# apache/arrow-rs

Measured on NVIDIA H100. Metric: Mrows/sec filter+take+add on 1e9-row Int64/Float64; % HBM roofline, higher is better.
Workload: dtype i64 (filter/take/sum) + f64 (add)

## Files before the change

### arrow-rs_b200/csrc/common.cuh

```cuda
#pragma once

#include <cuda_runtime.h>
#include <stdint.h>
#include <string.h>

#include <functional>
#include <unordered_map>
#include <vector>

#include "../../include/arrow_cuda.h"

#define ACU_FULL_MASK 0xffffffffu

enum {
  RES_COUNT = 0,
  RES_ERR_INDEX = 1,
  RES_AUX0 = 2,
  RES_AUX1 = 3,
  RES_AUX2 = 4,
  RES_AUX3 = 5,
  RES_ERR2 = 6,
  RES_SLOTS = 16,
  RES_BLOCKS = 64
};

struct acu_ctx {
  int device = 0;
  int sm_count = 0;
  cudaStream_t stream = nullptr;
  cudaEvent_t ev_start = nullptr, ev_stop = nullptr;
  acu_error_detail err{};
  int64_t launches = 0;
  int64_t bytes_allocated = 0;
  std::unordered_map<void *, size_t> allocs;
  std::unordered_map<const void *, int> occupancy;
  unsigned long long *d_res = nullptr;
  unsigned long long *h_res = nullptr;
  bool res_clean = false;
  int res_dirty_blocks = RES_BLOCKS;
  bool async_on = false;
  int async_blocks = 0;
  std::vector<std::function<acu_status(const unsigned long long *)>> async_fin;
  std::vector<int> async_blk;
  void *d_scratch = nullptr;
  size_t scratch_bytes = 0;
  void *nccl_comm = nullptr;
  int rank = 0, world = 1;
  cudaEvent_t tev[ACU_TIMER_SLOTS][2] = {};
  static constexpr int KEV_PAIRS = 64;
  cudaEvent_t kev[KEV_PAIRS][2] = {};
  int kev_class[KEV_PAIRS] = {};
  int kev_pending = 0;
  double kstat_ms[ACU_K_CLASSES] = {};
  int64_t kstat_n[ACU_K_CLASSES] = {};
};

void acu_kstats_drain(acu_ctx *ctx);
int acu_kstats_begin(acu_ctx *ctx, int cls);
void acu_kstats_end(acu_ctx *ctx, int slot);

acu_status acu_fail(acu_ctx *ctx, acu_status st, int64_t index, uint64_t lhs, uint64_t rhs,
                    uint64_t len, const char *fmt, ...) __attribute__((format(printf, 7, 8)));
acu_status acu_cuda_fail(acu_ctx *ctx, cudaError_t e, const char *what);
acu_status acu_scratch(acu_ctx *ctx, size_t bytes, void **out);
acu_status acu_res_reset(acu_ctx *ctx);
acu_status acu_res_fetch(acu_ctx *ctx);
acu_status acu_res_reset_n(acu_ctx *ctx, int blocks);
acu_status acu_res_fetch_n(acu_ctx *ctx, int blocks);
int acu_call_begin(acu_ctx *ctx, acu_status *st);
acu_status acu_call_end(acu_ctx *ctx, int block, std::function<acu_status(const unsigned long long *)> fin);
static inline unsigned long long *acu_dres(acu_ctx *ctx, int block) { return ctx->d_res + (size_t)block * RES_SLOTS; }
static inline const unsigned long long *acu_hres(const acu_ctx *ctx, int block) { return ctx->h_res + (size_t)block * RES_SLOTS; }
int64_t acu_resolve_null_count(acu_ctx *ctx, const acu_array *a, acu_status *st);

#define ACU_CUDA(ctx, expr)                                         \
  do {                                                              \
    cudaError_t _e = (expr);                                        \
    if (_e != cudaSuccess) return acu_cuda_fail((ctx), _e, #expr);  \
  } while (0)

#define ACU_ENTER(ctx)                                                                      \
  do {                                                                                      \
    cudaError_t _e = cudaSetDevice((ctx)->device);                                          \
    if (_e != cudaSuccess) return acu_cuda_fail((ctx), _e, "cudaSetDevice");                \
  } while (0)

#define ACU_TRY(expr)                  \
  do {                                 \
    acu_status _s = (expr);            \
    if (_s != ACU_OK) return _s;       \
  } while (0)

#define ACU_LAUNCH(ctx, kernel, grid, block, smem, ...)                            \
  do {                                                                             \
    kernel<<<(grid), (block), (smem), (ctx)->stream>>>(__VA_ARGS__);               \
    (ctx)->launches++;                                                             \
    cudaError_t _e = cudaGetLastError();                                           \
    if (_e != cudaSuccess) return acu_cuda_fail((ctx), _e, "launch " #kernel);     \
  } while (0)

#define ACU_LAUNCH_TIMED(ctx, cls, kernel, grid, block, smem, ...)                 \
  do {                                                                             \
    int _slot = acu_kstats_begin((ctx), (cls));                                    \
    kernel<<<(grid), (block), (smem), (ctx)->stream>>>(__VA_ARGS__);               \
    (ctx)->launches++;                                                             \
    cudaError_t _e = cudaGetLastError();                                           \
    acu_kstats_end((ctx), _slot);                                                  \
    if (_e != cudaSuccess) return acu_cuda_fail((ctx), _e, "launch " #kernel);     \
  } while (0)

static inline int acu_dtype_size(acu_dtype t) {
  switch (t) {
    case ACU_I8: case ACU_U8: return 1;
    case ACU_I16: case ACU_U16: return 2;
    case ACU_I32: case ACU_U32: case ACU_F32: return 4;
    default: return 8;
  }
}
static inline bool acu_dtype_is_float(acu_dtype t) { return t == ACU_F32 || t == ACU_F64; }
static inline bool acu_dtype_is_signed(acu_dtype t) { return t <= ACU_I64; }
static inline const char *acu_dtype_name(acu_dtype t) {
  static const char *n[] = {"Int8", "Int16", "Int32", "Int64", "UInt8", "UInt16", "UInt32", "UInt64", "Float32", "Float64"};
  return n[(int)t];
}

static inline int acu_grid(const acu_ctx *ctx, int64_t work_items, int per_sm) {
  int64_t g = (int64_t)ctx->sm_count * per_sm;
  if (g > work_items) g = work_items;
  if (g < 1) g = 1;
  return (int)g;
}

#ifdef __CUDACC__
template <class K>
static inline int acu_wave_grid(acu_ctx *ctx, K kernel, int block, size_t smem, int64_t work_blocks) {
  const void *key = reinterpret_cast<const void *>(kernel);
  auto it = ctx->occupancy.find(key);
  int per_sm;
  if (it == ctx->occupancy.end()) {
    per_sm = 0;
    if (cudaOccupancyMaxActiveBlocksPerMultiprocessor(&per_sm, kernel, block, smem) != cudaSuccess || per_sm < 1) per_sm = 1;
    ctx->occupancy[key] = per_sm;
  } else {
    per_sm = it->second;
  }
  return acu_grid(ctx, work_blocks, per_sm * 8);
}


__device__ __forceinline__ uint64_t ld_bits64(const uint8_t *__restrict__ base, int64_t pos, int64_t end) {
  int64_t n = end - pos;
  if (n <= 0) return 0ull;
  uintptr_t addr = (uintptr_t)base + (uintptr_t)(pos >> 3);
  uintptr_t al = addr & ~(uintptr_t)7;
  unsigned shift = (unsigned)((addr & 7) << 3) + (unsigned)(pos & 7);
  const uint64_t *p = reinterpret_cast<const uint64_t *>(al);
  uint64_t w = __ldg(p) >> shift;
  if (shift != 0 && (int64_t)(64 - shift) < n) w |= __ldg(p + 1) << (64 - shift);
  if (n < 64) w &= (~0ull) >> (64 - n);
  return w;
}

__device__ __forceinline__ uint32_t ld_bits32(const uint8_t *__restrict__ base, int64_t pos, int64_t end) {
  int64_t n = end - pos;
  if (n <= 0) return 0u;
  uintptr_t addr = (uintptr_t)base + (uintptr_t)(pos >> 3);
  uintptr_t al = addr & ~(uintptr_t)3;
  unsigned shift = (unsigned)((addr & 3) << 3) + (unsigned)(pos & 7);
  const uint32_t *p = reinterpret_cast<const uint32_t *>(al);
  uint32_t w = __ldg(p) >> shift;
  if (shift != 0 && (int64_t)(32 - shift) < n) w |= __ldg(p + 1) << (32 - shift);
  if (n < 32) w &= (~0u) >> (32 - n);
  return w;
}

__device__ __forceinline__ uint32_t ld_bit(const uint8_t *__restrict__ base, int64_t pos) {
  return (__ldg(base + (pos >> 3)) >> (pos & 7)) & 1u;
}

__device__ __forceinline__ uint4 ld_stream16(const void *p) {
  uint4 r;
  asm volatile("ld.global.nc.L1::no_allocate.v4.u32 {%0,%1,%2,%3}, [%4];"
               : "=r"(r.x), "=r"(r.y), "=r"(r.z), "=r"(r.w) : "l"(p));
  return r;
}
__device__ __forceinline__ void st_stream16(void *p, uint4 v) {
  asm volatile("st.global.cs.v4.u32 [%0], {%1,%2,%3,%4};" ::"l"(p), "r"(v.x), "r"(v.y), "r"(v.z), "r"(v.w) : "memory");
}
__device__ __forceinline__ uint64_t ld_stream8(const void *p) {
  uint64_t r;
  asm volatile("ld.global.nc.L1::no_allocate.u64 %0, [%1];" : "=l"(r) : "l"(p));
  return r;
}
__device__ __forceinline__ void st_stream8(void *p, uint64_t v) {
  asm volatile("st.global.cs.u64 [%0], %1;" ::"l"(p), "l"(v) : "memory");
}

template <class T> __device__ __forceinline__ T warp_sum(T v) {
#pragma unroll
  for (int o = 16; o > 0; o >>= 1) v += __shfl_xor_sync(ACU_FULL_MASK, v, o);
  return v;
}

__device__ __forceinline__ uint64_t splitmix64(uint64_t x) {
  x += 0x9E3779B97F4A7C15ull;
  x = (x ^ (x >> 30)) * 0xBF58476D1CE4E5B9ull;
  x = (x ^ (x >> 27)) * 0x94D049BB133111EBull;
  return x ^ (x >> 31);
}

__device__ __forceinline__ int64_t total_key(double x) {
  int64_t b = __double_as_longlong(x);
  return b ^ (int64_t)((uint64_t)(b >> 63) >> 1);
}
__device__ __forceinline__ int32_t total_key(float x) {
  int32_t b = __float_as_int(x);
  return b ^ (int32_t)((uint32_t)(b >> 31) >> 1);
}
#endif
```

### arrow-rs_b200/csrc/elementwise.cu

```cuda
#include <stdio.h>

#include <limits>
#include <type_traits>

#include "bitmap.cuh"

namespace {

template <class T, int EPL> struct alignas(EPL * sizeof(T) == 16 ? 16 : sizeof(T)) Pack { T v[EPL]; };

template <class T, int EPL>
__device__ __forceinline__ Pack<T, EPL> pack_load(const T *p) {
  Pack<T, EPL> r;
  if constexpr (EPL * sizeof(T) == 16) {
    uint4 x = ld_stream16(p);
    r = *reinterpret_cast<Pack<T, EPL> *>(&x);
  } else {
    static_assert(EPL == 1, "scalar path");
    r.v[0] = __ldg(p);
  }
  return r;
}
template <class T, int EPL>
__device__ __forceinline__ void pack_store(T *p, Pack<T, EPL> r) {
  if constexpr (EPL * sizeof(T) == 16) {
    st_stream16(p, *reinterpret_cast<uint4 *>(&r));
  } else {
    *p = r.v[0];
  }
}

__device__ __forceinline__ uint64_t ones_to(int64_t row, int64_t n) {
  int64_t k = n - row;
  return k >= 64 ? ~0ull : (k <= 0 ? 0ull : ((~0ull) >> (64 - k)));
}

enum { CLS_WRAP = 0, CLS_CHECKED = 1, CLS_DIVREM = 2 };
enum { OP_ADD = 0, OP_SUB = 1, OP_MUL = 2, OP_DIV = 3, OP_REM = 4, OP_NEG = 5 };

template <class T> struct is_fp { static constexpr bool value = std::is_floating_point<T>::value; };

__device__ __forceinline__ double fp_add(double a, double b) { return __dadd_rn(a, b); }
__device__ __forceinline__ double fp_sub(double a, double b) { return __dsub_rn(a, b); }
__device__ __forceinline__ double fp_mul(double a, double b) { return __dmul_rn(a, b); }
__device__ __forceinline__ double fp_div(double a, double b) { return __ddiv_rn(a, b); }
__device__ __forceinline__ double fp_rem(double a, double b) { return fmod(a, b); }
__device__ __forceinline__ float fp_add(float a, float b) { return __fadd_rn(a, b); }
__device__ __forceinline__ float fp_sub(float a, float b) { return __fsub_rn(a, b); }
__device__ __forceinline__ float fp_mul(float a, float b) { return __fmul_rn(a, b); }
__device__ __forceinline__ float fp_div(float a, float b) { return __fdiv_rn(a, b); }
__device__ __forceinline__ float fp_rem(float a, float b) { return fmodf(a, b); }

template <class T, int CLS>
__device__ __forceinline__ bool apply_op(int op, T l, T r, T &o) {
  if constexpr (is_fp<T>::value) {
    if constexpr (CLS == CLS_DIVREM) {
      o = (op == OP_DIV) ? fp_div(l, r) : fp_rem(l, r);
    } else {
      o = (op == OP_ADD) ? fp_add(l, r) : (op == OP_SUB) ? fp_sub(l, r) : (op == OP_MUL) ? fp_mul(l, r) : -r;
    }
    return false;
  } else {
    using U = typename std::make_unsigned<T>::type;
    constexpr bool SIGNED = std::is_signed<T>::value;
    if constexpr (CLS == CLS_WRAP) {
      U a = (U)l, b = (U)r;
      o = (T)((op == OP_ADD) ? (U)(a + b) : (op == OP_SUB) ? (U)(a - b) : (op == OP_MUL) ? (U)(a * b) : (U)((U)0 - b));
      return false;
    } else if constexpr (CLS == CLS_CHECKED) {
      if constexpr (sizeof(T) < 8) {
        using W = typename std::conditional<SIGNED, int64_t, uint64_t>::type;
        W a = (W)l, b = (W)r;
        W w = (op == OP_ADD) ? a + b : (op == OP_SUB) ? a - b : (op == OP_MUL) ? a * b : (W)0 - b;
        o = (T)w;
        if constexpr (SIGNED) return w < (W)std::numeric_limits<T>::min() || w > (W)std::numeric_limits<T>::max();
        else return (op == OP_SUB) ? (a < b) : (op == OP_NEG ? false : w > (W)std::numeric_limits<T>::max());
      } else if constexpr (SIGNED) {
        int64_t a = l, b = r;
        if (op == OP_NEG) { a = 0; }
        if (op == OP_ADD) {
          int64_t s = (int64_t)((uint64_t)a + (uint64_t)b);
          o = s;
          return ((a ^ s) & (b ^ s)) < 0;
        } else if (op == OP_MUL) {
          int64_t lo = (int64_t)((uint64_t)a * (uint64_t)b);
          int64_t hi = __mul64hi(a, b);
          o = lo;
          return hi != (lo >> 63);
        } else {
          int64_t s = (int64_t)((uint64_t)a - (uint64_t)b);
          o = s;
          return ((a ^ b) & (a ^ s)) < 0;
        }
      } else {
        uint64_t a = l, b = r;
        if (op == OP_ADD) { o = a + b; return o < a; }
        if (op == OP_MUL) { o = a * b; return __umul64hi(a, b) != 0; }
        if (op == OP_NEG) { o = (uint64_t)0 - b; return false; }
        o = a - b;
        return a < b;
      }
    } else {
      o = 0;
      if (r == 0) return true;
      if constexpr (SIGNED) {
        if (r == (T)-1) {
          if (op == OP_DIV) {
            if (l == std::numeric_limits<T>::min()) return true;
            o = (T)(-l);
          }
          return false;
        }
      }
      o = (op == OP_DIV) ? (T)(l / r) : (T)(l % r);
      return false;
    }
  }
}

template <class T>
struct ArithParams {
  const T *a, *b;
  T *out;
  int64_t n;
  const uint8_t *av, *bv;
  int64_t aoff, boff;
  uint64_t *out_valid;
  unsigned long long *res;
  int op;
  int a_scalar, b_scalar;
  int zero_nulls;
};

template <class T, int CLS, int EPL>
__global__ void __launch_bounds__(256, (CLS == CLS_WRAP ? 4 : 3)) k_arith(const ArithParams<T> p) {
  constexpr int R = (32 * EPL > 64) ? 32 * EPL : 64;
  constexpr int LPS = R / (32 * EPL);
  constexpr int U = (LPS >= 2) ? 2 : 4;
  constexpr int GROUP = U * R;
  constexpr int SG = 2048;
  constexpr int GPS = SG / GROUP;
  constexpr bool fallible = (CLS != CLS_WRAP) && !is_fp<T>::value;
  const int lane = threadIdx.x & 31;
  const int64_t warp = ((int64_t)blockIdx.x * blockDim.x + threadIdx.x) >> 5;
  const int64_t nwarps = ((int64_t)gridDim.x * blockDim.x) >> 5;
  const int64_t n = p.n;
  const int64_t sgroups = n / SG;
  const bool has_valid = p.out_valid != nullptr;
  T sa = T(), sb = T();
  if (p.a_scalar) sa = __ldg(p.a);
  if (p.b_scalar) sb = __ldg(p.b);
  unsigned valid_cnt = 0;
  unsigned long long err = ~0ull;

  for (int64_t sg = warp; sg < sgroups; sg += nwarps) {
    const int64_t sbase = sg * SG;
    uint64_t vw = ~0ull;
    if (has_valid) {
      const int64_t row = sbase + lane * 64;
      if (p.av) vw &= ld_bits64(p.av, p.aoff + row, p.aoff + n);
      if (p.bv) vw &= ld_bits64(p.bv, p.boff + row, p.boff + n);
      p.out_valid[row >> 6] = vw;
      valid_cnt += __popcll(vw);
    }
#pragma unroll 1
    for (int gi = 0; gi < GPS; ++gi) {
      const int64_t base = sbase + gi * GROUP;
      const T *__restrict__ pa = p.a + base + lane * EPL;
      const T *__restrict__ pb = p.b + base + lane * EPL;
      Pack<T, EPL> va[U * LPS], vb[U * LPS];
#pragma unroll
      for (int k = 0; k < U * LPS; ++k) {
        if (!p.a_scalar) va[k] = pack_load<T, EPL>(pa + k * 32 * EPL);
        if (!p.b_scalar) vb[k] = pack_load<T, EPL>(pb + k * 32 * EPL);
      }
      T *__restrict__ po = p.out + base + lane * EPL;
#pragma unroll
      for (int k = 0; k < U * LPS; ++k) {
        uint32_t bits = ~0u;
        if (fallible && p.zero_nulls) {
          const int pos = gi * GROUP + k * 32 * EPL + lane * EPL;
          const uint64_t w = __shfl_sync(ACU_FULL_MASK, vw, pos >> 6);
          bits = (uint32_t)(w >> (pos & 63));
        }
        Pack<T, EPL> o;
#pragma unroll
        for (int e = 0; e < EPL; ++e) {
          const T l = p.a_scalar ? sa : va[k].v[e];
          const T r = p.b_scalar ? sb : vb[k].v[e];
          T x;
          const bool bad = apply_op<T, CLS>(p.op, l, r, x);
          if (fallible) {
            if (!((bits >> e) & 1u)) x = T();
            else if (bad) {
              const unsigned long long i = (unsigned long long)(base + k * 32 * EPL + lane * EPL + e);
              err = i < err ? i : err;
            }
          }
          o.v[e] = x;
        }
        pack_store<T, EPL>(po + k * 32 * EPL, o);
      }
    }
  }

  if (warp == 0) {
    for (int64_t row = sgroups * SG; row < n; row += 64) {
      uint64_t vw = ones_to(row, n);
      if (has_valid) {
        if (p.av) vw &= ld_bits64(p.av, p.aoff + row, p.aoff + n);
        if (p.bv) vw &= ld_bits64(p.bv, p.boff + row, p.boff + n);
        if (lane == 0) { p.out_valid[row >> 6] = vw; valid_cnt += __popcll(vw); }
      }
#pragma unroll
      for (int h = 0; h < 2; ++h) {
        const int64_t i = row + h * 32 + lane;
        if (i >= n) continue;
        const T l = p.a_scalar ? sa : __ldg(p.a + i);
        const T r = p.b_scalar ? sb : __ldg(p.b + i);
        T x;
        const bool bad = apply_op<T, CLS>(p.op, l, r, x);
        if (fallible) {
          const bool live = !p.zero_nulls || ((vw >> (h * 32 + lane)) & 1ull);
          if (!live) x = T();
          else if (bad) err = (unsigned long long)i < err ? (unsigned long long)i : err;
        }
        p.out[i] = x;
      }
    }
  }
  if (has_valid) {
    valid_cnt = warp_sum(valid_cnt);
    if (lane == 0 && valid_cnt) atomicAdd(p.res + RES_COUNT, (unsigned long long)valid_cnt);
  }
  if (fallible && err != ~0ull) atomicMin(p.res + RES_ERR_INDEX, err);
}

template <class T, int CLS>
acu_status launch_arith(acu_ctx *ctx, const ArithParams<T> &p) {
  constexpr int EPLV = 16 / sizeof(T);
  bool aligned = ((uintptr_t)p.out % 16 == 0) && (p.a_scalar || (uintptr_t)p.a % 16 == 0) &&
                 (p.b_scalar || (uintptr_t)p.b % 16 == 0);
  if (aligned) {
    int64_t blocks = (p.n / 2048 + 1 + 7) / 8;
    ACU_LAUNCH_TIMED(ctx, ACU_K_ARITH, (k_arith<T, CLS, EPLV>), acu_wave_grid(ctx, k_arith<T, CLS, EPLV>, 256, 0, blocks), 256, 0, p);
  } else {
    int64_t blocks = (p.n / 2048 + 1 + 7) / 8;
    ACU_LAUNCH_TIMED(ctx, ACU_K_ARITH, (k_arith<T, CLS, 1>), acu_wave_grid(ctx, k_arith<T, CLS, 1>, 256, 0, blocks), 256, 0, p);
  }
  return ACU_OK;
}

const char *op_symbol(acu_arith_op op) {
  switch (op) {
    case ACU_ADD_WRAPPING: case ACU_ADD: return "+";
    case ACU_SUB_WRAPPING: case ACU_SUB: return "-";
    case ACU_MUL_WRAPPING: case ACU_MUL: return "*";
    case ACU_DIV: return "/";
    default: return "%";
  }
}

template <class T> void fmt_native(char *buf, size_t n, T v) {
  if constexpr (std::is_floating_point<T>::value) snprintf(buf, n, "%.17g", (double)v);
  else if constexpr (std::is_signed<T>::value) snprintf(buf, n, "%lld", (long long)v);
  else snprintf(buf, n, "%llu", (unsigned long long)v);
}
template <class T> uint64_t bits_of(T v) { uint64_t b = 0; memcpy(&b, &v, sizeof(T)); return b; }

template <class T>
acu_status arith_error(acu_ctx *ctx, acu_arith_op op, bool is_neg, const acu_array *a, const acu_array *b, int64_t idx) {
  T l = T(), r = T();
  if (a) ACU_CUDA(ctx, cudaMemcpyAsync(&l, static_cast<const T *>(a->values) + (a->is_scalar ? 0 : idx), sizeof(T), cudaMemcpyDeviceToHost, ctx->stream));
  ACU_CUDA(ctx, cudaMemcpyAsync(&r, static_cast<const T *>(b->values) + (b->is_scalar ? 0 : idx), sizeof(T), cudaMemcpyDeviceToHost, ctx->stream));
  ACU_CUDA(ctx, cudaStreamSynchronize(ctx->stream));
  char ls[40], rs[40];
  fmt_native(ls, sizeof ls, l);
  fmt_native(rs, sizeof rs, r);
  if (is_neg)
    return acu_fail(ctx, ACU_ERR_ARITHMETIC_OVERFLOW, idx, bits_of(r), 0, 0, "Overflow happened on: - %s", rs);
  if ((op == ACU_DIV || op == ACU_REM) && r == T())
    return acu_fail(ctx, ACU_ERR_DIVIDE_BY_ZERO, idx, bits_of(l), bits_of(r), 0, "Divide by zero error");
  return acu_fail(ctx, ACU_ERR_ARITHMETIC_OVERFLOW, idx, bits_of(l), bits_of(r), 0,
                  "Overflow happened on: %s %s %s", ls, op_symbol(op), rs);
}

acu_status set_new_null(acu_ctx *ctx, int64_t len, size_t value_bytes, acu_array_out *out) {
  if (value_bytes) ACU_CUDA(ctx, cudaMemsetAsync(out->values, 0, value_bytes, ctx->stream));
  if (len) ACU_CUDA(ctx, cudaMemsetAsync(out->validity, 0, acu_bitmap_bytes(len), ctx->stream));
  ACU_CUDA(ctx, cudaStreamSynchronize(ctx->stream));
  out->len = len;
  out->has_validity = 1;
  out->null_count = len;
  return ACU_OK;
}

template <class T>
acu_status arith_typed(acu_ctx *ctx, acu_arith_op op, const acu_array *a, const acu_array *b, acu_array_out *out) {
  const bool checked = !is_fp<T>::value && (op == ACU_ADD || op == ACU_SUB || op == ACU_MUL || op == ACU_DIV || op == ACU_REM);
  const bool a_s = a->is_scalar != 0, b_s = b->is_scalar != 0;
  acu_status st;
  ArithParams<T> p{};
  p.a = static_cast<const T *>(a->values);
  p.b = static_cast<const T *>(b->values);
  p.out = static_cast<T *>(out->values);
  p.res = ctx->d_res;
  p.a_scalar = a_s && !b_s;
  p.b_scalar = b_s && !a_s;
  switch (op) {
    case ACU_ADD_WRAPPING: case ACU_ADD: p.op = OP_ADD; break;
    case ACU_SUB_WRAPPING: case ACU_SUB: p.op = OP_SUB; break;
    case ACU_MUL_WRAPPING: case ACU_MUL: p.op = OP_MUL; break;
    case ACU_DIV: p.op = OP_DIV; break;
    default: p.op = OP_REM; break;
  }
  out->has_validity = 0;
  out->null_count = 0;
  int64_t len;
  if (a_s != b_s) {
    const acu_array *s = a_s ? a : b, *arr = a_s ? b : a;
    len = arr->len;
    int64_t snc = acu_resolve_null_count(ctx, s, &st);
    ACU_TRY(st);
    if (snc != 0) return set_new_null(ctx, len, (size_t)len * sizeof(T), out);
    out->len = len;
    if (len == 0) { out->has_validity = arr->validity != nullptr; return ACU_OK; }
    if (arr->validity) {
      (a_s ? p.bv : p.av) = arr->validity;
      (a_s ? p.boff : p.aoff) = arr->validity_offset;
      p.out_valid = reinterpret_cast<uint64_t *>(out->validity);
      p.zero_nulls = checked;
    }
  } else {
    if (a->len != b->len)
      return acu_fail(ctx, ACU_ERR_COMPUTE, -1, 0, 0, 0,
                      checked ? "Cannot perform a binary operation on arrays of different length"
                              : "Cannot perform binary operation on arrays of different length");
    len = a->len;
    out->len = len;
    if (len == 0) return ACU_OK;
    int64_t an = acu_resolve_null_count(ctx, a, &st);
    ACU_TRY(st);
    int64_t bn = acu_resolve_null_count(ctx, b, &st);
    ACU_TRY(st);
    if (a->validity && b->validity && (an > 0 || bn > 0)) {
      p.av = a->validity; p.aoff = a->validity_offset;
      p.bv = b->validity; p.boff = b->validity_offset;
    } else if (a->validity && !b->validity && an > 0) {
      p.av = a->validity; p.aoff = a->validity_offset;
    } else if (b->validity && !a->validity && bn > 0) {
      p.bv = b->validity; p.boff = b->validity_offset;
    }
    if (p.av || p.bv) {
      p.out_valid = reinterpret_cast<uint64_t *>(out->validity);
      p.zero_nulls = checked;
    }
  }
  p.n = len;
  const int blk = acu_call_begin(ctx, &st);
  ACU_TRY(st);
  p.res = acu_dres(ctx, blk);
  if (is_fp<T>::value) {
    if (op == ACU_DIV || op == ACU_REM) ACU_TRY((launch_arith<T, CLS_DIVREM>(ctx, p)));
    else ACU_TRY((launch_arith<T, CLS_WRAP>(ctx, p)));
  } else if (op == ACU_DIV || op == ACU_REM) {
    ACU_TRY((launch_arith<T, CLS_DIVREM>(ctx, p)));
  } else if (checked) {
    ACU_TRY((launch_arith<T, CLS_CHECKED>(ctx, p)));
  } else {
    ACU_TRY((launch_arith<T, CLS_WRAP>(ctx, p)));
  }
  const acu_array ca = *a, cb = *b;
  const bool has_valid = p.out_valid != nullptr;
  return acu_call_end(ctx, blk, [ctx, op, checked, ca, cb, has_valid, len, out](const unsigned long long *h) -> acu_status {
    if (checked && h[RES_ERR_INDEX] != ~0ull) return arith_error<T>(ctx, op, false, &ca, &cb, (int64_t)h[RES_ERR_INDEX]);
    if (has_valid) {
      out->has_validity = 1;
      out->null_count = len - (int64_t)h[RES_COUNT];
    }
    return ACU_OK;
  });
}

template <class T>
acu_status neg_typed(acu_ctx *ctx, int32_t checked_in, const acu_array *a, acu_array_out *out) {
  const bool checked = checked_in && !is_fp<T>::value;
  int64_t len = a->len;
  out->len = len;
  out->has_validity = a->validity != nullptr;
  out->null_count = 0;
  if (len == 0) return ACU_OK;
  ArithParams<T> p{};
  p.a = static_cast<const T *>(a->values);
  p.b = static_cast<const T *>(a->values);
  p.out = static_cast<T *>(out->values);
  p.res = ctx->d_res;
  p.a_scalar = 1;
  p.op = OP_NEG;
  p.n = len;
  if (a->validity) {
    p.bv = a->validity;
    p.boff = a->validity_offset;
    p.out_valid = reinterpret_cast<uint64_t *>(out->validity);
    p.zero_nulls = checked;
  }
  ACU_TRY(acu_res_reset(ctx));
  if (checked) ACU_TRY((launch_arith<T, CLS_CHECKED>(ctx, p)));
  else ACU_TRY((launch_arith<T, CLS_WRAP>(ctx, p)));
  ACU_TRY(acu_res_fetch(ctx));
  if (checked && ctx->h_res[RES_ERR_INDEX] != ~0ull)
    return arith_error<T>(ctx, ACU_SUB, true, nullptr, a, (int64_t)ctx->h_res[RES_ERR_INDEX]);
  if (p.out_valid) out->null_count = len - (int64_t)ctx->h_res[RES_COUNT];
  return ACU_OK;
}

enum { FOLD_NONE = 0, FOLD_DISTINCT = 1, FOLD_NOT_DISTINCT = 2 };

template <class T>
struct CmpParams {
  const T *a, *b;
  int64_t n;
  const uint8_t *av, *bv;
  int64_t aoff, boff;
  int a_scalar, b_scalar;
  int a_null_scalar, b_null_scalar;
  int neg, fold;
  uint64_t *out_bits, *out_valid;
  unsigned long long *res;
  int fuse;
  uint32_t *tile_count;
};

template <class T> __device__ __forceinline__ bool pred_eq(T l, T r) {
  if constexpr (sizeof(T) == 8 && is_fp<T>::value) return __double_as_longlong(l) == __double_as_longlong(r);
  else if constexpr (is_fp<T>::value) return __float_as_int(l) == __float_as_int(r);
  else return l == r;
}
template <class T> __device__ __forceinline__ bool pred_lt(T l, T r) {
  if constexpr (is_fp<T>::value) return total_key(l) < total_key(r);
  else return l < r;
}

template <class T, bool LT>
__global__ void __launch_bounds__(256) k_cmp(const CmpParams<T> p) {
  constexpr int U = 4;
  const int lane = threadIdx.x & 31;
  const int64_t warp = ((int64_t)blockIdx.x * blockDim.x + threadIdx.x) >> 5;
  const int64_t nwarps = ((int64_t)gridDim.x * blockDim.x) >> 5;
  const int64_t n = p.n;
  const int64_t strips = (n + 63) >> 6;
  T sa = T(), sb = T();
  if (p.a_scalar) sa = __ldg(p.a);
  if (p.b_scalar) sb = __ldg(p.b);
  unsigned valid_cnt = 0;
  for (int64_t s0 = warp * U; s0 < strips; s0 += nwarps * U) {
    T va[U][2], vb[U][2];
#pragma unroll
    for (int u = 0; u < U; ++u) {
#pragma unroll
      for (int h = 0; h < 2; ++h) {
        const int64_t i = (s0 + u) * 64 + h * 32 + lane;
        va[u][h] = (!p.a_scalar && i < n) ? __ldg(p.a + i) : sa;
        vb[u][h] = (!p.b_scalar && i < n) ? __ldg(p.b + i) : sb;
      }
    }
#pragma unroll
    for (int u = 0; u < U; ++u) {
      const int64_t row = (s0 + u) * 64;
      if (row >= n) break;
      bool r0 = LT ? pred_lt(va[u][0], vb[u][0]) : pred_eq(va[u][0], vb[u][0]);
      bool r1 = LT ? pred_lt(va[u][1], vb[u][1]) : pred_eq(va[u][1], vb[u][1]);
      uint64_t v = (uint64_t)__ballot_sync(ACU_FULL_MASK, r0) | ((uint64_t)__ballot_sync(ACU_FULL_MASK, r1) << 32);
      if (p.neg) v = ~v;
      if (lane == 0) {
        const uint64_t m = ones_to(row, n);
        v &= m;
        uint64_t l = p.a_null_scalar ? 0ull : m, r = p.b_null_scalar ? 0ull : m;
        if (p.av) l &= ld_bits64(p.av, p.aoff + row, p.aoff + n);
        if (p.bv) r &= ld_bits64(p.bv, p.boff + row, p.boff + n);
        if (p.fold == FOLD_DISTINCT) v = (l ^ r) | (l & r & v);
        else if (p.fold == FOLD_NOT_DISTINCT) v = (~(l | r) & m) | (l & r & v);
        else if (p.fuse) v &= l & r;
        p.out_bits[row >> 6] = v;
        if (p.out_valid) {
          p.out_valid[row >> 6] = l & r;
          valid_cnt += __popcll(l & r);
        }
      }
    }
  }
  if (p.out_valid && lane == 0 && valid_cnt) atomicAdd(p.res + RES_COUNT, (unsigned long long)valid_cnt);
}

template <class T, bool LT>
__global__ void __launch_bounds__(256, 4) k_cmp_v2(const CmpParams<T> p, const int64_t sgroups) {
  constexpr int EPL = 16 / sizeof(T);
  constexpr int RPL = 32 * EPL;
  constexpr int HPL = RPL / 32;
  constexpr int LOADS = 2048 / RPL;
  constexpr int U = LOADS < 4 ? LOADS : 4;
  const int lane = threadIdx.x & 31;
  const int64_t warp = ((int64_t)blockIdx.x * blockDim.x + threadIdx.x) >> 5;
  const int64_t nwarps = ((int64_t)gridDim.x * blockDim.x) >> 5;
  const int64_t n = p.n;
  T sa = T(), sb = T();
  if (p.a_scalar) sa = __ldg(p.a);
  if (p.b_scalar) sb = __ldg(p.b);
  unsigned valid_cnt = 0;
  const int grp_shift = (lane * EPL) & 31;
  const int grp_half = (lane * EPL) >> 5;
  for (int64_t sg = warp; sg < sgroups; sg += nwarps) {
    const int64_t sbase = sg << 11;
    uint64_t lw = ~0ull, rw = ~0ull;
    if (p.a_null_scalar) lw = 0;
    if (p.b_null_scalar) rw = 0;
    const int64_t wrow = sbase + lane * 64;
    if (p.av) lw &= ld_bits64(p.av, p.aoff + wrow, p.aoff + n);
    if (p.bv) rw &= ld_bits64(p.bv, p.boff + wrow, p.boff + n);
    uint32_t my_lo = 0, my_hi = 0;
#pragma unroll 1
    for (int l0 = 0; l0 < LOADS; l0 += U) {
      Pack<T, EPL> va[U], vb[U];
#pragma unroll
      for (int u = 0; u < U; ++u) {
        const int64_t i0 = sbase + (int64_t)(l0 + u) * RPL + lane * EPL;
        if (!p.a_scalar) va[u] = pack_load<T, EPL>(p.a + i0);
        if (!p.b_scalar) vb[u] = pack_load<T, EPL>(p.b + i0);
      }
#pragma unroll
      for (int u = 0; u < U; ++u) {
        uint32_t x = 0;
#pragma unroll
        for (int e = 0; e < EPL; ++e) {
          const T l = p.a_scalar ? sa : va[u].v[e];
          const T r = p.b_scalar ? sb : vb[u].v[e];
          x |= (uint32_t)(LT ? pred_lt(l, r) : pred_eq(l, r)) << e;
        }
        x <<= grp_shift;
#pragma unroll
        for (int hh = 0; hh < HPL; ++hh) {
          const uint32_t half = __reduce_or_sync(ACU_FULL_MASK, grp_half == hh ? x : 0u);
          const int widx = ((l0 + u) * HPL + hh) >> 1;
          if (lane == widx) { if (hh & 1) my_hi = half; else my_lo = half; }
        }
      }
// ... 395 lines not shown
```

### arrow-rs_b200/csrc/take.cu

```cuda
#include <stdio.h>
#include <stdlib.h>

#include <type_traits>

#include "bitmap.cuh"
#include "internal.cuh"

#define TAKE_WTILE_DEFAULT 256

namespace {

__device__ __forceinline__ uint32_t smem_u32(const void *p) { return (uint32_t)__cvta_generic_to_shared(p); }
__device__ __forceinline__ void mbar_init(uint64_t *bar, unsigned count) {
  asm volatile("mbarrier.init.shared::cta.b64 [%0], %1;" ::"r"(smem_u32(bar)), "r"(count) : "memory");
}
__device__ __forceinline__ void mbar_expect_tx(uint64_t *bar, unsigned bytes) {
  asm volatile("mbarrier.arrive.expect_tx.shared::cta.b64 _, [%0], %1;" ::"r"(smem_u32(bar)), "r"(bytes) : "memory");
}
__device__ __forceinline__ void mbar_wait(uint64_t *bar, unsigned parity) {
  asm volatile(
      "{\n"
      ".reg .pred p;\n"
      "WAIT_LOOP:\n"
      "mbarrier.try_wait.parity.shared::cta.b64 p, [%0], %1;\n"
      "@p bra DONE;\n"
      "bra WAIT_LOOP;\n"
      "DONE:\n"
      "}\n" ::"r"(smem_u32(bar)),
      "r"(parity)
      : "memory");
}
__device__ __forceinline__ void bulk_g2s(void *dst_smem, const void *src_gmem, unsigned bytes, uint64_t *bar) {
  asm volatile("cp.async.bulk.shared::cluster.global.mbarrier::complete_tx::bytes [%0], [%1], %2, [%3];" ::"r"(smem_u32(dst_smem)),
               "l"(src_gmem), "r"(bytes), "r"(smem_u32(bar))
               : "memory");
}

template <int W> struct VecOf;
template <> struct VecOf<1> { using type = uint8_t; };
template <> struct VecOf<2> { using type = uint16_t; };
template <> struct VecOf<4> { using type = uint32_t; };
template <> struct VecOf<8> { using type = uint64_t; };
template <> struct VecOf<16> { using type = uint4; };
struct alignas(16) U32B { uint4 lo, hi; };
template <> struct VecOf<32> { using type = U32B; };

template <class V> __device__ __forceinline__ V zero_of() { V v; memset(&v, 0, sizeof(V)); return v; }
template <class V> __device__ __forceinline__ V gather_ld(const V *p) {
  if constexpr (sizeof(V) == 32) {
    V v;
    v.lo = __ldg(reinterpret_cast<const uint4 *>(p));
    v.hi = __ldg(reinterpret_cast<const uint4 *>(p) + 1);
    return v;
  } else {
    return __ldg(p);
  }
}

struct TakeArgs {
  const void *values;
  int64_t n_values;
  const uint8_t *vvalid;
  int64_t vvoff;
  const uint8_t *vbits;
  int64_t vboff;
  const void *idx;
  int64_t m;
  const uint8_t *ivalid;
  int64_t ivoff;
  int idx_has_nulls;
  void *out;
  uint32_t *out_valid;
  uint32_t *out_bits;
  unsigned long long *res;
  int use_bulk;
};

template <int IT> struct IdxOf;
template <> struct IdxOf<0> { using raw = uint8_t; };
template <> struct IdxOf<1> { using raw = int8_t; };
template <> struct IdxOf<2> { using raw = uint16_t; };
template <> struct IdxOf<3> { using raw = int16_t; };
template <> struct IdxOf<4> { using raw = uint32_t; };
template <> struct IdxOf<5> { using raw = uint64_t; };
template <int IT> struct WideOf { using type = typename std::conditional<IT == 5, uint64_t, uint32_t>::type; };
template <int IT> __device__ __forceinline__ typename WideOf<IT>::type widen(typename IdxOf<IT>::raw v) {
  if constexpr (IT == 1 || IT == 3) return (uint32_t)(int32_t)v;
  else return (typename WideOf<IT>::type)v;
}

constexpr int TAKE_BATCH_COLS = 8;
struct TakeBatch { TakeArgs col[TAKE_BATCH_COLS]; };

template <int W, int IT, bool BOOL, int PL = 8, int MINB = 3>
__global__ void __launch_bounds__(256, MINB) k_take(const TakeBatch batch) {
  constexpr int TAKE_WTILE = 32 * PL;
  constexpr int TAKE_PER_LANE = PL;
  const TakeArgs a = batch.col[blockIdx.y];
  using V = typename VecOf<W>::type;
  using I = typename IdxOf<IT>::raw;
  __shared__ __align__(16) I s_idx[8][2][TAKE_WTILE];
  __shared__ __align__(8) uint64_t s_bar[8][2];
  const int lane = threadIdx.x & 31, wid = threadIdx.x >> 5;
  const int64_t warp = ((int64_t)blockIdx.x * blockDim.x + threadIdx.x) >> 5;
  const int64_t nwarps = ((int64_t)gridDim.x * blockDim.x) >> 5;
  const I *idx = static_cast<const I *>(a.idx);
  const int64_t n_tiles = (a.m + TAKE_WTILE - 1) / TAKE_WTILE;
  const bool gather_values = !BOOL && a.values != nullptr;
  unsigned valid_cnt = 0;
  unsigned long long err = ~0ull;

  if (lane == 0) { mbar_init(&s_bar[wid][0], 1); mbar_init(&s_bar[wid][1], 1); }
  asm volatile("fence.mbarrier_init.release.cluster;" ::: "memory");
  __syncwarp();

  auto stage = [&](int64_t t, int b) {
    const int64_t j0 = t * TAKE_WTILE;
    const int cnt = (int)((a.m - j0) < TAKE_WTILE ? (a.m - j0) : TAKE_WTILE);
    const bool bulk = a.use_bulk && cnt == TAKE_WTILE;
    if (bulk) {
      if (lane == 0) {
        mbar_expect_tx(&s_bar[wid][b], (unsigned)(TAKE_WTILE * sizeof(I)));
        bulk_g2s(&s_idx[wid][b][0], idx + j0, (unsigned)(TAKE_WTILE * sizeof(I)), &s_bar[wid][b]);
      }
    } else {
      for (int k = lane; k < cnt; k += 32) s_idx[wid][b][k] = __ldg(idx + j0 + k);
    }
    return bulk;
  };

  unsigned phase0 = 0, phase1 = 0;
  int64_t t = warp;
  bool cur_bulk = false;
  if (t < n_tiles) cur_bulk = stage(t, 0);
  int buf = 0;
  for (; t < n_tiles; t += nwarps) {
    const int64_t tn = t + nwarps;
    bool next_bulk = false;
    if (tn < n_tiles) next_bulk = stage(tn, buf ^ 1);
    if (cur_bulk) {
      mbar_wait(&s_bar[wid][buf], buf ? phase1 : phase0);
      if (buf) phase1 ^= 1; else phase0 ^= 1;
    }
    else __syncwarp();

    const int64_t j0 = t * TAKE_WTILE;
    typename WideOf<IT>::type ix[TAKE_PER_LANE];
    bool live[TAKE_PER_LANE], inb[TAKE_PER_LANE];
    V v[TAKE_PER_LANE];
    uint32_t bit[TAKE_PER_LANE];
#pragma unroll
    for (int k = 0; k < TAKE_PER_LANE; ++k) {
      const int j = k * 32 + lane;
      live[k] = j0 + j < a.m;
      ix[k] = live[k] ? widen<IT>(s_idx[wid][buf][j]) : 0;
      inb[k] = live[k] && (uint64_t)ix[k] < (uint64_t)a.n_values;
    }
#pragma unroll
    for (int k = 0; k < TAKE_PER_LANE; ++k) {
      if (gather_values) v[k] = inb[k] ? gather_ld<V>(static_cast<const V *>(a.values) + ix[k]) : zero_of<V>();
      uint32_t b = 1u;
      if (a.vvalid) b = inb[k] ? ld_bit(a.vvalid, a.vvoff + (int64_t)ix[k]) : 0u;
      if (BOOL) b |= (inb[k] ? ld_bit(a.vbits, a.vboff + (int64_t)ix[k]) : 0u) << 1;
      bit[k] = b;
    }
#pragma unroll
    for (int k = 0; k < TAKE_PER_LANE; ++k) {
      const int64_t gj = j0 + k * 32 + lane;
      uint32_t iv = ~0u;
      if (a.ivalid) iv = ld_bits32(a.ivalid, a.ivoff + (gj - lane), a.ivoff + a.m);
      const bool idx_valid = live[k] && ((iv >> lane) & 1u);
      const bool counts_as_valid_idx = a.idx_has_nulls ? idx_valid : live[k];
      if (live[k] && !inb[k] && counts_as_valid_idx) { unsigned long long e = (unsigned long long)gj; err = e < err ? e : err; }
      if (gather_values && live[k]) static_cast<V *>(a.out)[gj] = v[k];
      if (a.out_valid) {
        bool ob = live[k];
        if (a.vvalid) ob = ob && (bit[k] & 1u) && counts_as_valid_idx;
        else ob = idx_valid;
        const uint32_t word = __ballot_sync(ACU_FULL_MASK, ob);
        if (lane == 0 && gj < a.m) { a.out_valid[gj >> 5] = word; valid_cnt += __popc(word); }
      }
      if (BOOL) {
        const bool ob = live[k] && counts_as_valid_idx && ((bit[k] >> 1) & 1u);
        const uint32_t word = __ballot_sync(ACU_FULL_MASK, ob);
        if (lane == 0 && gj < a.m) a.out_bits[gj >> 5] = word;
      }
    }
    __syncwarp();
    buf ^= 1;
    cur_bulk = next_bulk;
  }
  if (a.out_valid) {
    if (lane == 0 && valid_cnt) atomicAdd(a.res + RES_COUNT, (unsigned long long)valid_cnt);
  }
  if (err != ~0ull) atomicMin(a.res + RES_ERR_INDEX, err);
}

template <int IT, bool SIGNED>
__global__ void __launch_bounds__(256) k_check_bounds(const void *idx_v, int64_t m, int64_t len,
                                                      const uint8_t *ivalid, int64_t ivoff,
                                                      unsigned long long *res) {
  using I = typename IdxOf<IT>::raw;
  const I *idx = static_cast<const I *>(idx_v);
  unsigned long long err = ~0ull;
  const int64_t stride = (int64_t)gridDim.x * blockDim.x;
  for (int64_t j = (int64_t)blockIdx.x * blockDim.x + threadIdx.x; j < m; j += stride) {
    if (ivalid && !ld_bit(ivalid, ivoff + j)) continue;
    bool bad;
    if constexpr (SIGNED) {
      using S = typename std::make_signed<I>::type;
      const int64_t v = (int64_t)(S)idx[j];
      bad = ivalid ? (v >= len) : (v < 0 || v >= len);
    } else {
      bad = (uint64_t)idx[j] >= (uint64_t)len;
    }
    if (bad && (unsigned long long)j < err) err = (unsigned long long)j;
  }
  if (err != ~0ull) atomicMin(res + RES_ERR_INDEX, err);
}

int index_kind(acu_dtype t) {
  switch (t) {
    case ACU_U8: return 0; case ACU_I8: return 1; case ACU_U16: return 2; case ACU_I16: return 3;
    case ACU_U32: case ACU_I32: return 4; case ACU_U64: case ACU_I64: return 5;
    default: return -1;
  }
}
uint64_t index_max(acu_dtype t) {
  switch (t) {
    case ACU_I8: return INT8_MAX; case ACU_I16: return INT16_MAX; case ACU_I32: return INT32_MAX;
    case ACU_I64: return INT64_MAX; case ACU_U8: return UINT8_MAX; case ACU_U16: return UINT16_MAX;
    case ACU_U32: return UINT32_MAX; default: return UINT64_MAX;
  }
}

template <int W>
acu_status launch_take_w(acu_ctx *ctx, int kind, const TakeBatch &tb, int n_cols) {
  const TakeArgs &ta = tb.col[0];
  constexpr int TAKE_WTILE = TAKE_WTILE_DEFAULT;
  const int64_t tiles = ((ta.m + TAKE_WTILE - 1) / TAKE_WTILE + 7) / 8;
#define ACU_TAKE_CASE(IT)                                                                                   \
  case IT:                                                                                                                   \
    if (W == 1 && ta.vbits)                                                                                                  \
      ACU_LAUNCH_TIMED(ctx, ACU_K_TAKE, (k_take<1, IT, true>), dim3(acu_wave_grid(ctx, k_take<1, IT, true>, 256, 0, tiles), n_cols), 256, 0, tb); \
    else                                                                                                                     \
      ACU_LAUNCH_TIMED(ctx, ACU_K_TAKE, (k_take<W, IT, false>), dim3(acu_wave_grid(ctx, k_take<W, IT, false>, 256, 0, tiles), n_cols), 256, 0, tb); \
    break;
  switch (kind) {
    ACU_TAKE_CASE(0) ACU_TAKE_CASE(1) ACU_TAKE_CASE(2) ACU_TAKE_CASE(3) ACU_TAKE_CASE(4) ACU_TAKE_CASE(5)
    default: break;
  }
#undef ACU_TAKE_CASE
  return ACU_OK;
}

acu_status launch_take(acu_ctx *ctx, int elem_bytes, int kind, const TakeBatch &tb, int n_cols) {
  switch (elem_bytes) {
    case 1: return launch_take_w<1>(ctx, kind, tb, n_cols);
    case 2: return launch_take_w<2>(ctx, kind, tb, n_cols);
    case 4: return launch_take_w<4>(ctx, kind, tb, n_cols);
    case 8: return launch_take_w<8>(ctx, kind, tb, n_cols);
    case 16: return launch_take_w<16>(ctx, kind, tb, n_cols);
    case 32: return launch_take_w<32>(ctx, kind, tb, n_cols);
    default: return acu_fail(ctx, ACU_ERR_INVALID_ARGUMENT, -1, 0, 0, 0, "take: unsupported element width %d", elem_bytes);
  }
}

acu_status fetch_index(acu_ctx *ctx, const acu_array *indices, acu_dtype t, int64_t j, uint64_t *raw, char *text, size_t n) {
  uint64_t v = 0;
  const int sz = acu_dtype_size(t);
  ACU_CUDA(ctx, cudaMemcpyAsync(&v, static_cast<const uint8_t *>(indices->values) + (size_t)j * sz, sz, cudaMemcpyDeviceToHost, ctx->stream));
  ACU_CUDA(ctx, cudaStreamSynchronize(ctx->stream));
  *raw = v;
  if (acu_dtype_is_signed(t)) {
    int64_t s = sz == 1 ? (int8_t)v : sz == 2 ? (int16_t)v : sz == 4 ? (int32_t)v : (int64_t)v;
    snprintf(text, n, "%lld", (long long)s);
  } else {
    snprintf(text, n, "%llu", (unsigned long long)v);
  }
  return ACU_OK;
}

}

acu_status acu_take_common(acu_ctx *ctx, int32_t elem_bytes, const acu_array *values, bool boolean_values,
                           const acu_array *indices, acu_dtype index_dtype, int32_t check_bounds,
                           acu_array_out *out) {
  ACU_ENTER(ctx);
  const int kind = index_kind(index_dtype);
  if (kind < 0)
    return acu_fail(ctx, ACU_ERR_INVALID_ARGUMENT, -1, 0, 0, 0, "Take only supported for integers, got %s", acu_dtype_name(index_dtype));
  acu_status st;
  const int64_t m = indices->len;
  const int64_t inc = acu_resolve_null_count(ctx, indices, &st);
  ACU_TRY(st);
  const bool idx_nulls = indices->validity && inc > 0;
  if (check_bounds) ACU_TRY(acu_take_check_bounds(ctx, indices, index_dtype, idx_nulls, values->len));
  out->len = m;
  out->has_validity = 0;
  out->null_count = 0;
  if (m == 0) return ACU_OK;
  const int64_t vnc = acu_resolve_null_count(ctx, values, &st);
  ACU_TRY(st);
  const bool val_nulls = values->validity && vnc > 0;
  int mode = 0;
  const int blk = acu_call_begin(ctx, &st);
  ACU_TRY(st);
  ACU_TRY(acu_take_col_launch(ctx, elem_bytes, values, boolean_values, val_nulls, indices, index_dtype, idx_nulls, out, acu_dres(ctx, blk), &mode));
  const acu_array v = *values, ix = *indices;
  return acu_call_end(ctx, blk, [ctx, v, ix, index_dtype, mode, out](const unsigned long long *h) -> acu_status {
    return acu_take_col_finalize(ctx, &v, &ix, index_dtype, mode, h, out);
  });
}

static TakeArgs take_args(int32_t elem_bytes, const acu_array *values, bool boolean_values, bool val_nulls, const acu_array *indices,
                          acu_dtype , bool idx_nulls, acu_array_out *out, unsigned long long *res) {
  TakeArgs ta{};
  ta.values = (elem_bytes > 0 && !boolean_values) ? values->values : nullptr;
  ta.n_values = values->len;
  if (val_nulls) { ta.vvalid = values->validity; ta.vvoff = values->validity_offset; }
  if (boolean_values) { ta.vbits = static_cast<const uint8_t *>(values->values); ta.vboff = values->values_offset; ta.out_bits = static_cast<uint32_t *>(out->values); }
  ta.idx = indices->values;
  ta.m = indices->len;
  if (idx_nulls || (!val_nulls && indices->validity)) { ta.ivalid = indices->validity; ta.ivoff = indices->validity_offset; }
  ta.idx_has_nulls = idx_nulls;
  ta.out = out->values;
  if (val_nulls || indices->validity) ta.out_valid = reinterpret_cast<uint32_t *>(out->validity);
  ta.res = res;
  ta.use_bulk = ((uintptr_t)indices->values % 16) == 0;
  return ta;
}

acu_status acu_take_col_launch(acu_ctx *ctx, int32_t elem_bytes, const acu_array *values, bool boolean_values, bool val_nulls,
                               const acu_array *indices, acu_dtype index_dtype, bool idx_nulls, acu_array_out *out,
                               unsigned long long *res, int *mode) {
  *mode = 0;
  const int kind = index_kind(index_dtype);
  out->len = indices->len;
  out->has_validity = 0;
// ... 109 lines not shown
```

Measured before the change: 74670.

## Add TMA bulk-copy pipelined kernel for aligned wrapping array-array arithmetic

Adds a k_arith_bulk kernel that streams both input chunks into shared memory with cp.async.bulk and mbarriers, using a 3-stage ring so loads overlap compute and stores. A tail kernel handles rows beyond the last full 2048-row chunk. The mbarrier helpers move from take.cu into common.cuh so both files can share them. The per-chunk __syncthreads and the single issuing thread may limit throughput, and the 96KB of shared memory caps occupancy.

After: 76110, median of 6. 1.9% higher.

```diff
diff --git a/arrow-rs_b200/csrc/common.cuh b/arrow-rs_b200/csrc/common.cuh
--- a/arrow-rs_b200/csrc/common.cuh
+++ b/arrow-rs_b200/csrc/common.cuh
@@ -196,6 +196,32 @@
   asm volatile("st.global.cs.u64 [%0], %1;" ::"l"(p), "l"(v) : "memory");
 }
 
+__device__ __forceinline__ uint32_t smem_u32(const void *p) { return (uint32_t)__cvta_generic_to_shared(p); }
+__device__ __forceinline__ void mbar_init(uint64_t *bar, unsigned count) {
+  asm volatile("mbarrier.init.shared::cta.b64 [%0], %1;" ::"r"(smem_u32(bar)), "r"(count) : "memory");
+}
+__device__ __forceinline__ void mbar_expect_tx(uint64_t *bar, unsigned bytes) {
+  asm volatile("mbarrier.arrive.expect_tx.shared::cta.b64 _, [%0], %1;" ::"r"(smem_u32(bar)), "r"(bytes) : "memory");
+}
+__device__ __forceinline__ void mbar_wait(uint64_t *bar, unsigned parity) {
+  asm volatile(
+      "{\n"
+      ".reg .pred p;\n"
+      "WAIT_LOOP:\n"
+      "mbarrier.try_wait.parity.shared::cta.b64 p, [%0], %1;\n"
+      "@p bra DONE;\n"
+      "bra WAIT_LOOP;\n"
+      "DONE:\n"
+      "}\n" ::"r"(smem_u32(bar)),
+      "r"(parity)
+      : "memory");
+}
+__device__ __forceinline__ void bulk_g2s(void *dst_smem, const void *src_gmem, unsigned bytes, uint64_t *bar) {
+  asm volatile("cp.async.bulk.shared::cluster.global.mbarrier::complete_tx::bytes [%0], [%1], %2, [%3];" ::"r"(smem_u32(dst_smem)),
+               "l"(src_gmem), "r"(bytes), "r"(smem_u32(bar))
+               : "memory");
+}
+
 template <class T> __device__ __forceinline__ T warp_sum(T v) {
 #pragma unroll
   for (int o = 16; o > 0; o >>= 1) v += __shfl_xor_sync(ACU_FULL_MASK, v, o);
diff --git a/arrow-rs_b200/csrc/elementwise.cu b/arrow-rs_b200/csrc/elementwise.cu
--- a/arrow-rs_b200/csrc/elementwise.cu
+++ b/arrow-rs_b200/csrc/elementwise.cu
@@ -236,11 +236,104 @@
   if (fallible && err != ~0ull) atomicMin(p.res + RES_ERR_INDEX, err);
 }
 
+constexpr int ARITH_BULK_ROWS = 2048;
+constexpr int ARITH_BULK_STAGES = 3;
+template <class T> constexpr size_t arith_bulk_smem() {
+  return (size_t)ARITH_BULK_STAGES * 2 * ARITH_BULK_ROWS * sizeof(T) + ARITH_BULK_STAGES * sizeof(uint64_t);
+}
+
+template <class T>
+__global__ void __launch_bounds__(256, 2) k_arith_bulk(const ArithParams<T> p) {
+  constexpr int EPL = 16 / sizeof(T);
+  constexpr int CH = ARITH_BULK_ROWS, S = ARITH_BULK_STAGES;
+  constexpr unsigned CB = CH * sizeof(T);
+  extern __shared__ __align__(128) unsigned char smem[];
+  uint64_t *bar = reinterpret_cast<uint64_t *>(smem + (size_t)S * 2 * CB);
+  const int lane = threadIdx.x & 31, wid = threadIdx.x >> 5;
+  const int64_t chunks = p.n / CH;
+  const bool has_valid = p.out_valid != nullptr;
+  if (threadIdx.x == 0) {
+    for (int s = 0; s < S; ++s) mbar_init(&bar[s], 1);
+    asm volatile("fence.mbarrier_init.release.cluster;" ::: "memory");
+  }
+  __syncthreads();
+  auto issue = [&](int64_t c, int s) {
+    mbar_expect_tx(&bar[s], 2 * CB);
+    bulk_g2s(smem + (size_t)s * 2 * CB, p.a + c * CH, CB, &bar[s]);
+    bulk_g2s(smem + (size_t)s * 2 * CB + CB, p.b + c * CH, CB, &bar[s]);
+  };
+  if (threadIdx.x == 0)
+    for (int s = 0; s < S; ++s)
+      if (blockIdx.x + (int64_t)s * gridDim.x < chunks) issue(blockIdx.x + (int64_t)s * gridDim.x, s);
+  unsigned valid_cnt = 0;
+  int it = 0;
+  for (int64_t c = blockIdx.x; c < chunks; c += gridDim.x, ++it) {
+    const int s = it % S;
+    const bool vwarp = has_valid && wid == (it & 7);
+    uint64_t vw = ~0ull;
+    const int64_t vrow = c * CH + lane * 64;
+    if (vwarp) {
+      if (p.av) vw &= ld_bits64(p.av, p.aoff + vrow, p.aoff + p.n);
+      if (p.bv) vw &= ld_bits64(p.bv, p.boff + vrow, p.boff + p.n);
+    }
+    mbar_wait(&bar[s], (unsigned)(it / S) & 1u);
+    const Pack<T, EPL> *sa = reinterpret_cast<const Pack<T, EPL> *>(smem + (size_t)s * 2 * CB);
+    const Pack<T, EPL> *sb = reinterpret_cast<const Pack<T, EPL> *>(smem + (size_t)s * 2 * CB + CB);
+#pragma unroll
+    for (int k = 0; k < (CH / EPL + 255) / 256; ++k) {
+      const int v = threadIdx.x + k * 256;
+      if ((CH / EPL) % 256 != 0 && v >= CH / EPL) break;
+      const Pack<T, EPL> x = sa[v], y = sb[v];
+      Pack<T, EPL> o;
+#pragma unroll
+      for (int e = 0; e < EPL; ++e) apply_op<T, CLS_WRAP>(p.op, x.v[e], y.v[e], o.v[e]);
+      pack_store<T, EPL>(p.out + c * CH + v * EPL, o);
+    }
+    if (vwarp) {
+      p.out_valid[vrow >> 6] = vw;
+      valid_cnt += __popcll(vw);
+    }
+    __syncthreads();
+    if (threadIdx.x == 0 && c + (int64_t)S * gridDim.x < chunks) issue(c + (int64_t)S * gridDim.x, s);
+  }
+  if (has_valid) {
+    valid_cnt = warp_sum(valid_cnt);
+    if (lane == 0 && valid_cnt) atomicAdd(p.res + RES_COUNT, (unsigned long long)valid_cnt);
+  }
+}
+
 template <class T, int CLS>
 acu_status launch_arith(acu_ctx *ctx, const ArithParams<T> &p) {
   constexpr int EPLV = 16 / sizeof(T);
   bool aligned = ((uintptr_t)p.out % 16 == 0) && (p.a_scalar || (uintptr_t)p.a % 16 == 0) &&
                  (p.b_scalar || (uintptr_t)p.b % 16 == 0);
+  const int64_t chunks = p.n / ARITH_BULK_ROWS;
+  if (CLS == CLS_WRAP && aligned && !p.a_scalar && !p.b_scalar && chunks > 0) {
+    constexpr size_t smem = arith_bulk_smem<T>();
+    ACU_CUDA(ctx, cudaFuncSetAttribute(k_arith_bulk<T>, cudaFuncAttributeMaxDynamicSharedMemorySize, (int)smem));
+    const void *key = reinterpret_cast<const void *>(k_arith_bulk<T>);
+    auto itc = ctx->occupancy.find(key);
+    int per_sm = 0;
+    if (itc == ctx->occupancy.end()) {
+      if (cudaOccupancyMaxActiveBlocksPerMultiprocessor(&per_sm, k_arith_bulk<T>, 256, smem) != cudaSuccess || per_sm < 1) per_sm = 1;
+      ctx->occupancy[key] = per_sm;
+    } else {
+      per_sm = itc->second;
+    }
+    ACU_LAUNCH_TIMED(ctx, ACU_K_ARITH, (k_arith_bulk<T>), acu_grid(ctx, chunks, per_sm), 256, smem, p);
+    const int64_t head = chunks * ARITH_BULK_ROWS;
+    if (head == p.n) return ACU_OK;
+    ArithParams<T> q = p;
+    q.a += head;
+    q.b += head;
+    q.out += head;
+    q.aoff += head;
+    q.boff += head;
+    if (q.out_valid) q.out_valid += head >> 6;
+    q.n = p.n - head;
+    ACU_LAUNCH_TIMED(ctx, ACU_K_ARITH, (k_arith<T, CLS, EPLV>), 1, 256, 0, q);
+    return ACU_OK;
+  }
   if (aligned) {
     int64_t blocks = (p.n / 2048 + 1 + 7) / 8;
     ACU_LAUNCH_TIMED(ctx, ACU_K_ARITH, (k_arith<T, CLS, EPLV>), acu_wave_grid(ctx, k_arith<T, CLS, EPLV>, 256, 0, blocks), 256, 0, p);
diff --git a/arrow-rs_b200/csrc/take.cu b/arrow-rs_b200/csrc/take.cu
--- a/arrow-rs_b200/csrc/take.cu
+++ b/arrow-rs_b200/csrc/take.cu
@@ -9,32 +9,6 @@
 #define TAKE_WTILE_DEFAULT 256
 
 namespace {
-
-__device__ __forceinline__ uint32_t smem_u32(const void *p) { return (uint32_t)__cvta_generic_to_shared(p); }
-__device__ __forceinline__ void mbar_init(uint64_t *bar, unsigned count) {
-  asm volatile("mbarrier.init.shared::cta.b64 [%0], %1;" ::"r"(smem_u32(bar)), "r"(count) : "memory");
-}
-__device__ __forceinline__ void mbar_expect_tx(uint64_t *bar, unsigned bytes) {
-  asm volatile("mbarrier.arrive.expect_tx.shared::cta.b64 _, [%0], %1;" ::"r"(smem_u32(bar)), "r"(bytes) : "memory");
-}
-__device__ __forceinline__ void mbar_wait(uint64_t *bar, unsigned parity) {
-  asm volatile(
-      "{\n"
-      ".reg .pred p;\n"
-      "WAIT_LOOP:\n"
-      "mbarrier.try_wait.parity.shared::cta.b64 p, [%0], %1;\n"
-      "@p bra DONE;\n"
-      "bra WAIT_LOOP;\n"
-      "DONE:\n"
-      "}\n" ::"r"(smem_u32(bar)),
-      "r"(parity)
-      : "memory");
-}
-__device__ __forceinline__ void bulk_g2s(void *dst_smem, const void *src_gmem, unsigned bytes, uint64_t *bar) {
-  asm volatile("cp.async.bulk.shared::cluster.global.mbarrier::complete_tx::bytes [%0], [%1], %2, [%3];" ::"r"(smem_u32(dst_smem)),
-               "l"(src_gmem), "r"(bytes), "r"(smem_u32(bar))
-               : "memory");
-}
 
 template <int W> struct VecOf;
 template <> struct VecOf<1> { using type = uint8_t; };
```
